# jenkinsm13/julia-spira

Hardware: AMD Instinct MI355X
Metric: Msamples/sec at 1920x1080 spp=64 depth=8; fraction of HBM roofline (higher is better)
Workload: dtype f64

## Files before the change

### julia-spira_amd/csrc/spira_device.h

```cpp
#pragma once
#include <hip/hip_runtime.h>
#include <stdint.h>
#include <type_traits>
#include "spira_fastdiv.h"

namespace spira {

__device__ __forceinline__ float sqrt_rn(float x) { return __builtin_sqrtf(x); }
__device__ __forceinline__ double sqrt_rn(double x) { return __builtin_sqrt(x); }

constexpr int kBlock = 256;
#ifndef SPIRA_WAVES_F32
#define SPIRA_WAVES_F32 5
#endif
#ifndef SPIRA_WAVES_F64
#define SPIRA_WAVES_F64 4
#endif
#define SPIRA_WAVES_PER_SIMD(T) (sizeof(T) == 8 ? SPIRA_WAVES_F64 : SPIRA_WAVES_F32)
constexpr uint32_t kMaxTries = 64;

template <class T> struct Vec { T x, y, z; };

template <class T> __device__ __forceinline__ Vec<T> mk(T x, T y, T z) { Vec<T> r; r.x = x; r.y = y; r.z = z; return r; }
template <class T> __device__ __forceinline__ Vec<T> operator+(Vec<T> a, Vec<T> b) { return mk<T>(a.x + b.x, a.y + b.y, a.z + b.z); }
// ... 870 lines not shown
template <class T>
__device__ __forceinline__ void dielectric_resolve(Pending<T> &pend, const Vec<T> d, const RngKey &key) {
    const Vec<T> n = pend.v;
    const T ior = pend.rough;
    const T cosd = dot(d, n);
    const bool entering = cosd < (T)0.0;
    const Vec<T> nn = entering ? n : mk<T>(-n.x, -n.y, -n.z);
    const T eta = entering ? (T)1.0 / ior : ior;
    const T ci = entering ? -cosd : cosd;
    const T s2 = (eta * eta) * ((T)1.0 - ci * ci);
    T r0 = ((T)1.0 - ior) / ((T)1.0 + ior); r0 = r0 * r0;
    const T x = (T)1.0 - ci, x2 = x * x;
    const T refl = r0 + ((T)1.0 - r0) * ((x2 * x2) * x);
    T u, u1, u2;
    rng3<T>(key, 1, u, u1, u2);
    if (s2 > (T)1.0 || u < refl) pend.v = d - nn * ((T)2 * dot(d, nn));
    else pend.v = d * eta + nn * (eta * ci - sqrt_rn((T)1.0 - s2));
    pend.kind = kMirror;
}

template <class T, bool BVH, bool EXT = false>
__device__ __forceinline__ SegInfo segment_front(const SceneLds<T> &sc, Vec<T> &o, const Vec<T> d, Vec<T> &beta, bool scatter,
                                                 Vec<T> &contrib, T &t_out, Pending<T> &pend, const ExtState<T> *ext = nullptr) {
    SegInfo info;
    T t;
    uint32_t slot;
    int prim = closest_hit<T, BVH>(sc, o, d, (T)0.001, t, slot);
    info.prim = prim;
    t_out = prim >= 0 ? t : (T)0;
    if (prim < 0) {
        pend.kind = kDead; pend.rough = 0; pend.v = mk<T>(0, 0, 0);
        contrib = sky_term_x<T, EXT>(d, beta, ext);
        info.alive = false; info.has_contrib = true;
        return info;
    }
    const Vec<T> pos = o + d * t;
    info.has_contrib = shade_hit<T, BVH, EXT>(sc, pos, d, prim, slot, beta, scatter, contrib, pend, ext);
    info.alive = scatter;
    if (scatter) o = pos;
    return info;
}

template <class T, class P>
__device__ __forceinline__ Vec<T> segment_back(const Vec<T> pos, const Pending<T> &pend, const Vec<T> rnd, P &pol) {
    if (pend.kind == kDiffuse) return normalize((pend.v + rnd) - pos, pol);
    Vec<T> reflected = pend.v;
    if (pend.kind == kSpecRough) reflected = reflected + rnd * pend.rough;
    return normalize(reflected, pol);
}
template <class T>
__device__ __forceinline__ Vec<T> segment_back(const Vec<T> pos, const Pending<T> &pend, const Vec<T> rnd) {
    ExactDiv exact;
    return segment_back<T>(pos, pend, rnd, exact);
}

template <class T, bool BVH, bool EXT = false>
__device__ __forceinline__ SegInfo trace_segment(const SceneLds<T> &sc, const RenderConst<T> &rc, Vec<T> &o, Vec<T> &d,
                                                 Vec<T> &beta, uint32_t pixel, uint32_t sample, uint32_t bounce,
                                                 bool scatter, Vec<T> &contrib, T &t_out, const ExtState<T> *ext = nullptr) {
    Pending<T> pend;
    const Vec<T> d_in = d;
    SegInfo info = segment_front<T, BVH, EXT>(sc, o, d, beta, scatter, contrib, t_out, pend, ext);
    if (info.alive) {
        Vec<T> rnd = mk<T>(0, 0, 0);
        if (EXT && pend.kind == kDielectric) dielectric_resolve<T>(pend, d_in, rng_key(rc.sA, rc.sB, pixel, sample, bounce));
        if (pend.kind == kDiffuse || pend.kind == kSpecRough)
            rnd = random_in_unit_sphere<T>(rng_key(rc.sA, rc.sB, pixel, sample, bounce));
        d = segment_back<T>(o, pend, rnd);
    }
    return info;
}

template <class T, class P>
__device__ __forceinline__ void camera_ray(const RenderConst<T> &rc, uint32_t i, uint32_t j, uint32_t pixel, uint32_t sample,
                                           Vec<T> &o, Vec<T> &d, P &pol) {
    T xu, xv, unused;
    rng3<T>(rng_key(rc.sA, rc.sB, pixel, sample, 0), 0, xu, xv, unused);
    T u = ((T)(i - 1) + xu) / (T)(rc.width - 1);
    T v = ((T)(j - 1) + xv) / (T)(rc.height - 1);
    o = rc.cam_origin;
    d = normalize(((rc.cam_llc + rc.cam_hor * u) + rc.cam_ver * v) - o, pol);
}
template <class T>
__device__ __forceinline__ void camera_ray(const RenderConst<T> &rc, uint32_t i, uint32_t j, uint32_t pixel, uint32_t sample,
                                           Vec<T> &o, Vec<T> &d) {
    ExactDiv exact;
    camera_ray<T>(rc, i, j, pixel, sample, o, d, exact);
}
__device__ __forceinline__ float to_scalar(float x) { return __uint_as_float(__builtin_amdgcn_readfirstlane(__float_as_uint(x))); }
__device__ __forceinline__ double to_scalar(double x) {
    const uint32_t lo = __builtin_amdgcn_readfirstlane((uint32_t)__double2loint(x)), hi = __builtin_amdgcn_readfirstlane((uint32_t)__double2hiint(x));
    return __hiloint2double((int)hi, (int)lo);
}
template <class T> struct PixelDiv { Recip<T> w1, h1; };
template <class T> __device__ __forceinline__ PixelDiv<T> pixel_divisors(const RenderConst<T> &rc) {
    PixelDiv<T> p;
    p.w1 = recip_of((T)(rc.width - 1)); p.h1 = recip_of((T)(rc.height - 1));
    p.w1.d = to_scalar(p.w1.d); p.w1.r = to_scalar(p.w1.r); p.h1.d = to_scalar(p.h1.d); p.h1.r = to_scalar(p.h1.r);
    return p;
}
template <class T> __device__ __forceinline__ T pixel_quotient(T n, const Recip<T> &rc, ExactDiv &) { return n / rc.d; }
template <class T> __device__ __forceinline__ T pixel_quotient(T n, const Recip<T> &rc, SpecDiv &) { return quotient(n, rc); }
template <class T, class P>
__device__ __forceinline__ void camera_ray_lds(const RenderConst<T> &rc, const T *cam, const PixelDiv<T> &pd, uint32_t i, uint32_t j, uint32_t pixel, uint32_t sample,
                                               Vec<T> &o, Vec<T> &d, P &pol) {
    T xu, xv, unused;
    rng3<T>(rng_key(rc.sA, rc.sB, pixel, sample, 0), 0, xu, xv, unused);
    T u = pixel_quotient<T>((T)(i - 1) + xu, pd.w1, pol);
    T v = pixel_quotient<T>((T)(j - 1) + xv, pd.h1, pol);
    o = mk<T>(cam[0], cam[1], cam[2]);
    const Vec<T> llc = mk<T>(cam[3], cam[4], cam[5]), hor = mk<T>(cam[6], cam[7], cam[8]), ver = mk<T>(cam[9], cam[10], cam[11]);
    d = normalize(((llc + hor * u) + ver * v) - o, pol);
}

template <class T>
__device__ __forceinline__ void path_of(const RenderConst<T> &rc, uint32_t q, uint32_t pass, uint32_t &i, uint32_t &j,
                                        uint32_t &pixel, uint32_t &sample) {
    uint32_t slot = fastdiv(q, rc.fd_tile);
    uint32_t pl = q - slot * rc.tile_pixels;
    uint32_t lr = fastdiv(pl, rc.fd_width);
    uint32_t lx = pl - lr * rc.width;
    j = ref_row_j(rc, lr);
    i = lx + 1;
    pixel = (j - 1) * rc.width + lx;
    sample = rc.sample0 + pass * rc.slots + slot;
}

template <class T> struct RayQueue { Pack4<T> *A; Pack4<T> *B; Pack2<T> *C; };

struct Stats {
    unsigned long long segments, rays_enqueued, radiance_rmw, radiance_store, redone_waves, rays_parked;
    unsigned long long mesh_wave_trips, mesh_lane_trips;
};

template <class T> struct BounceArgs {
    SceneGlobal<T> scene;
    RenderConst<T> rc;
    RayQueue<T> qin, qout;
    Pack3<T> *L;
    const uint32_t *cnt_in;
    uint32_t *cnt_out;
    uint32_t *blk_stats;
    uint32_t cap;
    Stats *stats;
    uint32_t bounce;
    uint32_t pass;
    uint32_t n_first;
};

__device__ __forceinline__ void wave_lds_sync() {
    __builtin_amdgcn_fence(__ATOMIC_RELEASE, "wavefront");
    __builtin_amdgcn_wave_barrier();
    __builtin_amdgcn_fence(__ATOMIC_ACQUIRE, "wavefront");
}

template <class T, bool FIRST, int R, bool BVH>
__global__ __launch_bounds__(kBlock, SPIRA_WAVES_PER_SIMD(T)) void k_bounce(const BounceArgs<T> a) {
    extern __shared__ __attribute__((aligned(32))) unsigned char lds_raw[];
    constexpr uint32_t WPB = kBlock / 64, SUB = 64 * R;
    const uint32_t lane = threadIdx.x & 63, wave = threadIdx.x >> 6;
    const uint32_t NW = gridDim.x * WPB, wid = blockIdx.x * WPB + wave;
    const RenderConst<T> &rc = a.rc;
    const bool scatter = (a.bounce + 1 < rc.max_depth);
    uint32_t n_mine = 0;
    if (!FIRST) {
        uint32_t n_blk = 0;
#pragma unroll
        for (uint32_t w = 0; w < WPB; ++w) n_blk += a.cnt_in[blockIdx.x * WPB + w];
        n_mine = a.cnt_in[wid];
        if (n_blk == 0) {
            if (lane == 0) { if (scatter) a.cnt_out[wid] = 0; a.blk_stats[4 * wid] = 0; a.blk_stats[4 * wid + 1] = 0; a.blk_stats[4 * wid + 2] = 0; a.blk_stats[4 * wid + 3] = 0; }
            return;
        }
    }
    const SceneLds<T> sc = stage_scene<T>(a.scene, lds_raw);
    Pack4<T> *s_rnd = reinterpret_cast<Pack4<T> *>(lds_raw + scene_lds_bytes<T>(a.scene.n_spheres, a.scene.n_materials, a.scene.n_triangles)) + wave * SUB;
    const uint32_t region = wid * a.cap;
    const unsigned long long lt_mask = (1ull << lane) - 1ull;
    uint32_t n_rmw = 0, n_store = 0, n_seg = 0, fill = 0;

    const uint32_t limit = FIRST ? a.n_first : n_mine;
    const uint32_t n_sub = (limit + SUB - 1) / SUB;
    for (uint32_t sub = FIRST ? wid : 0u; sub < n_sub; sub += FIRST ? NW : 1u) {
        Vec<T> o[R], beta[R];
        Pending<T> pend[R];
        uint32_t q[R], ent[R];
        uint32_t n_list = 0;
#pragma unroll
        for (int r = 0; r < R; ++r) {
            const uint32_t idx = sub * SUB + r * 64 + lane;
            pend[r].kind = kDead;
            bool want = false;
            RngKey key;
            if (idx < limit) {
                uint32_t pixel, sample, pi, pj;
                Vec<T> d;
                if (FIRST) {
                    q[r] = idx;
                    path_of<T>(rc, idx, a.pass, pi, pj, pixel, sample);
                    camera_ray<T>(rc, pi, pj, pixel, sample, o[r], d);
                    beta[r] = mk<T>(1, 1, 1);
                } else {
                    const Pack4<T> A = a.qin.A[region + idx], B = a.qin.B[region + idx];
                    const Pack2<T> C = a.qin.C[region + idx];
                    o[r] = mk<T>(A.x, A.y, A.z);
                    d = mk<T>(A.w, B.x, B.y);
                    beta[r] = mk<T>(B.z, B.w, C.x);
                    q[r] = Bits<T>::to_u32(C.y);
                }
                Vec<T> contrib; T t_hit;
                SegInfo si = segment_front<T, BVH>(sc, o[r], d, beta[r], scatter, contrib, t_hit, pend[r]);
                ++n_seg;
                const uint32_t qi = q[r] & 0x7FFFFFFFu;
                const bool has_l = (q[r] >> 31) != 0;
                if (si.has_contrib) {
                    Pack3<T> l; l.x = contrib.x; l.y = contrib.y; l.z = contrib.z;
                    if (has_l) { const Pack3<T> l0 = a.L[qi]; l.x = l0.x + contrib.x; l.y = l0.y + contrib.y; l.z = l0.z + contrib.z; ++n_rmw; }
                    else ++n_store;
                    a.L[qi] = l;
                    q[r] |= 0x80000000u;
                } else if (!si.alive && !has_l) {
                    Pack3<T> l; l.x = 0; l.y = 0; l.z = 0;
                    a.L[qi] = l;
                    ++n_store;
                }
                want = (pend[r].kind == kDiffuse || pend[r].kind == kSpecRough);
                if (want) {
                    if (!FIRST) path_of<T>(rc, qi, a.pass, pi, pj, pixel, sample);
                    key = rng_key(rc.sA, rc.sB, pixel, sample, a.bounce);
                }
            }
            if (scatter) {
                const unsigned long long m = __ballot(want);
                if (want) {
                    ent[r] = n_list + __popcll(m & lt_mask);
                    uint32_t *kw = reinterpret_cast<uint32_t *>(&s_rnd[ent[r]]);
                    kw[0] = key.hA; kw[1] = key.hB;
                }
                n_list += (uint32_t)__popcll(m);
            }
        }
        if (!scatter) continue;
        wave_lds_sync();
        {
            uint32_t e = lane, t = 1, next = 64;
            bool have = e < n_list;
            RngKey k; k.hA = 0; k.hB = 0; k.hBr = 0;
            if (have) {
                const uint32_t *kw = reinterpret_cast<const uint32_t *>(&s_rnd[e]);
                k.hA = kw[0]; k.hB = kw[1]; k.hBr = (k.hB << 16) | (k.hB >> 16);
            }
            while (__any(have)) {
                bool done = false;
                if (have) {
                    T u0, u1, u2;
                    rng3<T>(k, t, u0, u1, u2, (T)(1.0 / 1048576.0));
                    Vec<T> c = mk<T>(u0, u1, u2) - mk<T>(1, 1, 1);
                    done = dot(c, c) < (T)1.0;
                    if (!done && t == kMaxTries) { c = mk<T>(0, 0, 0); done = true; }
                    if (done) { Pack4<T> w; w.x = c.x; w.y = c.y; w.z = c.z; w.w = 0; s_rnd[e] = w; }
                    ++t;
                }
                const unsigned long long m = __ballot(done);
                if (done) {
                    e = next + __popcll(m & lt_mask); t = 1;
                    have = e < n_list;
                    if (have) {
                        const uint32_t *kw = reinterpret_cast<const uint32_t *>(&s_rnd[e]);
                        k.hA = kw[0]; k.hB = kw[1]; k.hBr = (k.hB << 16) | (k.hB >> 16);
                    }
                }
                next += (uint32_t)__popcll(m);
            }
        }
        wave_lds_sync();
#pragma unroll
        for (int r = 0; r < R; ++r) {
            const bool alive = pend[r].kind != kDead;
            const unsigned long long m = __ballot(alive);
            if (alive) {
                Vec<T> rnd = mk<T>(0, 0, 0);
                if (pend[r].kind != kMirror) { const Pack4<T> w = s_rnd[ent[r]]; rnd = mk<T>(w.x, w.y, w.z); }
                const Vec<T> nd = segment_back<T>(o[r], pend[r], rnd);
                const uint32_t dst = region + fill + __popcll(m & lt_mask);
                Pack4<T> A, B; Pack2<T> C;
                A.x = o[r].x; A.y = o[r].y; A.z = o[r].z; A.w = nd.x;
                B.x = nd.y; B.y = nd.z; B.z = beta[r].x; B.w = beta[r].y;
                C.x = beta[r].z; C.y = Bits<T>::from_u32(q[r]);
                a.qout.A[dst] = A; a.qout.B[dst] = B; a.qout.C[dst] = C;
            }
            fill += (uint32_t)__popcll(m);
        }
        wave_lds_sync();
    }
    for (int sft = 32; sft > 0; sft >>= 1) { n_rmw += __shfl_down(n_rmw, sft); n_seg += __shfl_down(n_seg, sft); n_store += __shfl_down(n_store, sft); }
    if (lane == 0) {
        if (scatter) a.cnt_out[wid] = fill;
        a.blk_stats[4 * wid] = n_seg;
        a.blk_stats[4 * wid + 1] = n_rmw;
        a.blk_stats[4 * wid + 2] = n_store;
        a.blk_stats[4 * wid + 3] = FIRST ? 0u : n_seg;
    }
}

template <class T> struct PathArgs {
    SceneGlobal<T> scene;
    RenderConst<T> rc;
    RayQueue<T> q[2];
    uint32_t *qref[2];
    uint2 *qkey[2];
    uint32_t cam_consts;
    Pack3<T> *L;
    uint32_t *blk_stats;
    uint32_t cap;
    uint32_t pass;
    uint32_t n_first;
    uint32_t dense_pct;
    Pack4<T> *mesh_list;
    uint32_t mesh_min_batch;
    uint32_t refill_free;
    uint32_t mesh_mode;
    uint32_t *mesh_count;
    uint32_t resume_k, resume_nw;
    uint32_t *redo;
    uint32_t redo_only;
    Stats *stats;
    Pack4<T> *accum;
    FastDiv fd_keff;
    uint32_t k_eff;
    uint32_t accum_first;
    uint32_t l_private;
};

#ifndef SPIRA_RESOLVE_RUN
#define SPIRA_RESOLVE_RUN 4
#endif
__device__ __forceinline__ uint32_t owned_pixel(uint32_t w, uint32_t nw, uint32_t l) {
    constexpr uint32_t kRun = SPIRA_RESOLVE_RUN;
    static_assert(64 % kRun == 0, "a run length divides the wave");
    return ((l / kRun) * nw + w) * kRun + l % kRun;
}

template <class T>
__device__ __forceinline__ void resolve_pixel(Pack4<T> *accum, const Pack3<T> *L, uint32_t tile_pixels, uint32_t k_eff, bool first_pass, uint32_t p) {
    Pack4<T> acc;
    if (first_pass) { acc.x = 0; acc.y = 0; acc.z = 0; acc.w = 0; } else acc = accum[p];
    uint32_t s = 0;
    for (; s + 8 <= k_eff; s += 8) {
        Pack3<T> l[8];
#pragma unroll
        for (int k = 0; k < 8; ++k) l[k] = L[(size_t)(s + k) * tile_pixels + p];
#pragma unroll
        for (int k = 0; k < 8; ++k) { acc.x = acc.x + l[k].x; acc.y = acc.y + l[k].y; acc.z = acc.z + l[k].z; }
    }
    for (; s < k_eff; ++s) {
        const Pack3<T> l = L[(size_t)s * tile_pixels + p];
        acc.x = acc.x + l.x; acc.y = acc.y + l.y; acc.z = acc.z + l.z;
    }
    accum[p] = acc;
}
template <class T>
__device__ __forceinline__ void resolve_pixel_run(Pack4<T> *accum, const Pack3<T> *Lp, uint32_t k_eff, bool first_pass, uint32_t p) {
    constexpr uint32_t kRun = SPIRA_RESOLVE_RUN;
    Pack4<T> acc;
    if (first_pass) { acc.x = 0; acc.y = 0; acc.z = 0; acc.w = 0; } else acc = accum[p];
    uint32_t s = 0;
    for (; s + 8 <= k_eff; s += 8) {
        Pack3<T> l[8];
#pragma unroll
        for (int k = 0; k < 8; ++k) l[k] = Lp[(s + k) * kRun];
#pragma unroll
        for (int k = 0; k < 8; ++k) { acc.x = acc.x + l[k].x; acc.y = acc.y + l[k].y; acc.z = acc.z + l[k].z; }
    }
    for (; s < k_eff; ++s) {
        const Pack3<T> l = Lp[s * kRun];
        acc.x = acc.x + l.x; acc.y = acc.y + l.y; acc.z = acc.z + l.z;
    }
    accum[p] = acc;
}

__device__ __forceinline__ float pack_qref(uint32_t q, uint32_t, float) { return __uint_as_float(q); }
__device__ __forceinline__ double pack_qref(uint32_t q, uint32_t ref, double) { return __longlong_as_double((long long)((unsigned long long)q | ((unsigned long long)ref << 32))); }
__device__ __forceinline__ uint32_t unpack_q(float w) { return __float_as_uint(w); }
__device__ __forceinline__ uint32_t unpack_q(double w) { return (uint32_t)(unsigned long long)__double_as_longlong(w); }
__device__ __forceinline__ uint32_t unpack_ref(double w) { return (uint32_t)((unsigned long long)__double_as_longlong(w) >> 32); }

#ifdef SPIRA_MESH_STATS
__device__ unsigned long long g_mesh_dbg[32];
#define MESH_STAT(...) __VA_ARGS__
#else
#define MESH_STAT(...)
#endif

#ifndef SPIRA_CARRY_KEY
#define SPIRA_CARRY_KEY 1
#endif
#ifndef SPIRA_WAVES_B_F32
#define SPIRA_WAVES_B_F32 4
#endif
#ifndef SPIRA_WAVES_B_F64
#define SPIRA_WAVES_B_F64 SPIRA_WAVES_F64
#endif
#ifndef SPIRA_WAVES_PATH_F32
#define SPIRA_WAVES_PATH_F32 6
#endif
template <class T, int R, bool BVH, bool EXT, bool SPEC, int MODE = 0, bool TRI = true>
__global__ __launch_bounds__(kBlock, MODE == 2 ? (sizeof(T) == 8 ? SPIRA_WAVES_B_F64 : SPIRA_WAVES_B_F32) : (sizeof(T) == 4 ? SPIRA_WAVES_PATH_F32 : SPIRA_WAVES_F64)) void k_path(const PathArgs<T> a) {
    extern __shared__ __attribute__((aligned(32))) unsigned char lds_raw[];
    constexpr uint32_t WPB = kBlock / 64, SUB = 64 * R;
    constexpr bool kRefArray = sizeof(T) == 4;
    constexpr bool kCarry = SPIRA_CARRY_KEY && !BVH && !EXT;
    constexpr uint32_t kStageShift = 25, kRefMask = (1u << kStageShift) - 1u;
    const uint32_t lane = threadIdx.x & 63, wave = threadIdx.x >> 6;
    const uint32_t NW = gridDim.x * WPB, wid = blockIdx.x * WPB + wave;
    const RenderConst<T> &rc = a.rc;
    using Pol = typename std::conditional<SPEC, SpecDiv, ExactDiv>::type;
    Pol pol;
    if (!SPEC && a.redo_only) {
        uint32_t any = 0;
        for (uint32_t w = 0; w < WPB; ++w) any |= a.redo[blockIdx.x * WPB + w];
        if (!any) return;
    }
    T *cam_lds = reinterpret_cast<T *>(lds_raw + scene_lds_bytes<T>(a.scene.n_spheres, a.scene.n_materials, a.scene.n_triangles) + WPB * SUB * sizeof(Pack4<T>));
    if (threadIdx.x < 12) {
        const Vec<T> *cv = threadIdx.x < 3 ? &rc.cam_origin : (threadIdx.x < 6 ? &rc.cam_llc : (threadIdx.x < 9 ? &rc.cam_hor : &rc.cam_ver));
        const uint32_t cc = threadIdx.x % 3;
        cam_lds[threadIdx.x] = cc == 0 ? cv->x : (cc == 1 ? cv->y : cv->z);
    }
    Pack4<T> *cam_sph = reinterpret_cast<Pack4<T> *>(reinterpret_cast<unsigned char *>(cam_lds) + 128);
    constexpr bool kCam = !EXT;
    if (kCam && MODE != 2 && a.cam_consts)
        for (uint32_t i = threadIdx.x; i < a.scene.n_spheres; i += blockDim.x) {
            const T *sp = a.scene.spheres5 + 5 * (size_t)i;
            const Vec<T> oc = rc.cam_origin - mk<T>(sp[0], sp[1], sp[2]);
            Pack4<T> k; k.x = oc.x; k.y = oc.y; k.z = oc.z; k.w = dot(oc, oc) - sp[3] * sp[3];
// ... 37 lines not shown
    uint32_t pfx[kMaxSeg + 1];
    bool segmented = false;
    {
        uint32_t cnt = 0;
        if (mesh_mode == 2u && lane < kseg && wid * kseg + lane < a.resume_nw) cnt = a.mesh_count[wid * kseg + lane];
        pfx[0] = 0;
#pragma unroll
        for (int j = 0; j < kMaxSeg; ++j) pfx[j + 1] = pfx[j] + (uint32_t)__builtin_amdgcn_readlane((int)cnt, j);
        if (mesh_mode == 2u) { mfill = pfx[kMaxSeg]; segmented = true; }
    }
    const uint32_t first_sub = own ? 0u : (mesh_mode == 1u ? (wid % a.resume_k) * (NW / a.resume_k) + wid / a.resume_k : wid);
    const uint32_t sub_step = own ? 1u : NW;
    MESH_STAT(unsigned long long dbg_t0 = __builtin_readcyclecounter(); unsigned long long dbg_sess = 0, dbg_walk = 0; uint32_t dbg_ns = 0, dbg_ws = 0, dbg_ls = 0, dbg_rf = 0, dbg_rays = 0, dbg_rounds = 0, dbg_ws1 = 0, dbg_ls1 = 0, dbg_h[4] = {0, 0, 0, 0};)
    for (uint32_t round = 0; ; ++round) {
        MESH_STAT(++dbg_rounds;)
        const bool first = mesh_mode != 2u && round == 0;
        const RayQueue<T> qin = a.q[(round + 1) & 1], qout = a.q[round & 1];
        const uint32_t *rin = a.qref[(round + 1) & 1];
        uint32_t *rout = a.qref[round & 1];
        const uint2 *kin = a.qkey[(round + 1) & 1];
        uint2 *kout = a.qkey[round & 1];
        const uint32_t limit = first ? (own ? n_own : a.n_first) : n_in;
        const uint32_t n_sub = first ? n_sub_first : (n_in + SUB - 1) / SUB;
        uint32_t fill = 0;
        for (uint32_t sub = first ? first_sub : 0u; sub < n_sub; sub += first ? sub_step : 1u) {
            Vec<T> o[R], beta[R];
            Pending<T> pend[R];
            ExtState<T> ex[R];
            uint32_t q[R], ent[R], stg[R], ref[R];
            uint32_t ka[R], kb[R];
            bool valid[R];
#pragma unroll
            for (int r = 0; r < R; ++r) {
                const uint32_t idx = sub * SUB + r * 64 + lane;
                valid[r] = false; stg[r] = round; ref[r] = 0; q[r] = 0; ka[r] = 0; kb[r] = 0;
                pend[r].kind = kDead; pend[r].rough = 0; pend[r].v = mk<T>(0, 0, 0);
                o[r] = mk<T>(0, 0, 0); beta[r] = mk<T>(1, 1, 1);
                bool parked = false; T park_t = 0; int park_prim = -1;
                uint32_t qf = idx;
                bool in = idx < limit;
                if (own && first) {
                    const uint32_t t = idx / SPIRA_RESOLVE_RUN, run = fastdiv(t, a.fd_keff);
                    const uint32_t px = owned_pixel(wid, NW, run * SPIRA_RESOLVE_RUN + idx % SPIRA_RESOLVE_RUN);
                    qf = (t - run * a.k_eff) * rc.tile_pixels + px;
                    in = in && px < rc.tile_pixels;
                }
                const uint32_t ql = priv ? l_base + idx : qf;
                if (in) {
                    if (first) {
                        uint32_t pixel, sample, pi, pj;
                        Vec<T> d;
                        q[r] = ql;
                        path_of<T>(rc, qf, a.pass, pi, pj, pixel, sample);
                        if (kCarry) { ka[r] = mix32(rc.sA + pixel) ^ (sample << 8); kb[r] = mix32(rc.sB ^ pixel) + (sample << 8); }
                        camera_ray_lds<T>(rc, cam_lds, pix_div, pi, pj, pixel, sample, o[r], d, pol);
                        if (EXT) { ex[r].flags = rc.flags; if (rc.flags & kExtSpectral) beta[r] = ext_wavelength<T>(sc, rc.sA, rc.sB, pixel, sample, ex[r]); }
                        T t; uint32_t slot = 0;
                        int prim;
                        if (defer) {
                            if (kCam && a.cam_consts) closest_hit_local<T, Pol, TRI, true>(sc, o[r], d, (T)0.001, t, prim, pol, cam_sph);
                            else closest_hit_local<T, Pol, TRI>(sc, o[r], d, (T)0.001, t, prim, pol);
                            parked = mesh_box_hit<T>(sc, o[r], d, t);
                        } else if (kCam && !BVH && a.cam_consts) { closest_hit_local<T, Pol, TRI, true>(sc, o[r], d, (T)0.001, t, prim, pol, cam_sph); }
                        else prim = closest_hit<T, BVH, Pol, TRI>(sc, o[r], d, (T)0.001, t, slot, pol);
                        ++n_seg;
                        if (parked) { park_t = t; park_prim = prim; pend[r].v = d; }
                        else if (prim < 0) {
                            const Vec<T> c = sky_term_x<T, EXT>(d, beta[r], &ex[r]);
                            Pack3<T> l; l.x = c.x; l.y = c.y; l.z = c.z;
                            a.L[ql] = l;
                            ++n_store;
                        } else {
                            valid[r] = true;
                            o[r] = o[r] + d * t;
                            ref[r] = (BVH && prim >= (int)ref_base) ? ref_base + slot : (uint32_t)prim;
                            pend[r].v = d;
                        }
                    } else {
                        const Pack4<T> A = qin.A[region + idx], B = qin.B[region + idx];
                        const Pack2<T> C = qin.C[region + idx];
                        o[r] = mk<T>(A.x, A.y, A.z);
                        pend[r].v = mk<T>(A.w, B.x, B.y);
                        beta[r] = mk<T>(B.z, B.w, C.x);
                        q[r] = unpack_q(C.y);
                        uint32_t w;
                        if constexpr (kRefArray) w = rin[region + idx]; else w = unpack_ref(C.y);
                        if (mixed) { stg[r] = w >> kStageShift; ref[r] = w & kRefMask; } else ref[r] = w;
                        if (kCarry) { const uint2 k = kin[region + idx]; ka[r] = k.x; kb[r] = k.y; }
                        valid[r] = true;
                    }
                }
                if (defer && first) {
                    const unsigned long long mp = __ballot(parked);
                    if (parked) park(mfill + __popcll(mp & lt_mask), o[r], pend[r].v, beta[r], park_t, q[r], park_prim, 0u);
                    mfill += (uint32_t)__popcll(mp); n_park += (uint32_t)__popcll(mp);
                }
            }
            while (true) {
                uint32_t n_list = 0, n_valid = 0;
#pragma unroll
                for (int r = 0; r < R; ++r) {
                    bool want = false;
                    RngKey key;
                    const Vec<T> d = pend[r].v;
                    pend[r].kind = kDead;
                    if (valid[r]) {
                        uint32_t pixel = 0, sample = 0, pi, pj;
                        const bool scatter = stg[r] + 1 < rc.max_depth;
                        int prim = (int)ref[r]; uint32_t slot = 0;
                        if (BVH && ref[r] >= ref_base) { prim = (int)ref_base; slot = ref[r] - ref_base; }
                        const uint32_t qi = q[r] & 0x7FFFFFFFu;
                        const bool has_l = (q[r] >> 31) != 0;
                        if (EXT) {
                            path_of<T>(rc, qi, a.pass, pi, pj, pixel, sample);
                            ex[r].flags = rc.flags;
                            if (rc.flags & kExtSpectral) (void)ext_wavelength<T>(sc, rc.sA, rc.sB, pixel, sample, ex[r]);
                        }
                        Vec<T> contrib;
                        const bool has_contrib = shade_hit<T, BVH, EXT, Pol, TRI>(sc, o[r], d, prim, slot, beta[r], scatter, contrib, pend[r], &ex[r], pol);
                        if (has_contrib) {
                            Pack3<T> l; l.x = contrib.x; l.y = contrib.y; l.z = contrib.z;
                            if (has_l) { const Pack3<T> l0 = a.L[qi]; l.x = l0.x + contrib.x; l.y = l0.y + contrib.y; l.z = l0.z + contrib.z; ++n_rmw; }
                            else ++n_store;
                            a.L[qi] = l;
                            q[r] |= 0x80000000u;
                        } else if (!scatter && !has_l) {
                            Pack3<T> l; l.x = 0; l.y = 0; l.z = 0;
                            a.L[qi] = l;
                            ++n_store;
                        }
                        want = (pend[r].kind == kDiffuse || pend[r].kind == kSpecRough);
                        if (want || (EXT && pend[r].kind == kDielectric)) {
                            if (kCarry && mixed) {
                                key.hA = mix32(ka[r] ^ stg[r]); key.hB = mix32(kb[r] + stg[r]); key.hBr = (key.hB << 16) | (key.hB >> 16);
                            } else {
                                if (!EXT) path_of<T>(rc, qi, a.pass, pi, pj, pixel, sample);
                                key = rng_key(rc.sA, rc.sB, pixel, sample, stg[r]);
                            }
                            if (EXT && pend[r].kind == kDielectric) dielectric_resolve<T>(pend[r], d, key);
                        }
                    }
                    const unsigned long long mv = __ballot(pend[r].kind != kDead);
                    n_valid += (uint32_t)__popcll(mv);
                    const unsigned long long m = __ballot(want);
                    if (want) {
                        ent[r] = n_list + __popcll(m & lt_mask);
                        uint32_t *kw = reinterpret_cast<uint32_t *>(&s_rnd[ent[r]]);
                        kw[0] = key.hA; kw[1] = key.hB;
                    }
                    n_list += (uint32_t)__popcll(m);
                }
                if (n_valid == 0) break;
                wave_lds_sync();
                {
                    uint32_t e = lane, t = 1, next = 64;
                    bool have = e < n_list;
                    RngKey k; k.hA = 0; k.hB = 0; k.hBr = 0;
                    if (have) {
                        const uint32_t *kw = reinterpret_cast<const uint32_t *>(&s_rnd[e]);
                        k.hA = kw[0]; k.hB = kw[1]; k.hBr = (k.hB << 16) | (k.hB >> 16);
                    }
                    while (__any(have)) {
                        bool done = false;
                        if (have) {
                            T u0, u1, u2;
                            rng3<T>(k, t, u0, u1, u2, (T)(1.0 / 1048576.0));
                            Vec<T> c = mk<T>(u0, u1, u2) - mk<T>(1, 1, 1);
                            done = dot(c, c) < (T)1.0;
                            if (!done && t == kMaxTries) { c = mk<T>(0, 0, 0); done = true; }
                            if (done) { Pack4<T> w; w.x = c.x; w.y = c.y; w.z = c.z; w.w = 0; s_rnd[e] = w; }
                            ++t;
                        }
                        const unsigned long long m = __ballot(done);
                        if (done) {
                            e = next + __popcll(m & lt_mask); t = 1;
                            have = e < n_list;
                            if (have) {
                                const uint32_t *kw = reinterpret_cast<const uint32_t *>(&s_rnd[e]);
                                k.hA = kw[0]; k.hB = kw[1]; k.hBr = (k.hB << 16) | (k.hB >> 16);
                            }
                        }
                        next += (uint32_t)__popcll(m);
                    }
                }
                wave_lds_sync();
                uint32_t n_hit = 0;
#pragma unroll
                for (int r = 0; r < R; ++r) {
                    bool hit = false, parked3 = false;
                    T park_t3 = 0; int park_prim3 = -1;
                    if (pend[r].kind != kDead) {
                        Vec<T> rnd = mk<T>(0, 0, 0);
                        if (pend[r].kind != kMirror) { const Pack4<T> w = s_rnd[ent[r]]; rnd = mk<T>(w.x, w.y, w.z); }
                        const Vec<T> nd = segment_back<T>(o[r], pend[r], rnd, pol);
                        T t; uint32_t slot = 0;
                        int prim;
                        if (defer) {
                            closest_hit_local<T, Pol, TRI>(sc, o[r], nd, (T)0.001, t, prim, pol);
                            parked3 = mesh_box_hit<T>(sc, o[r], nd, t);
                        } else prim = closest_hit<T, BVH, Pol, TRI>(sc, o[r], nd, (T)0.001, t, slot, pol);
                        ++n_seg;
                        if (parked3) { park_t3 = t; park_prim3 = prim; pend[r].v = nd; }
                        else if (prim < 0) {
                            const Vec<T> c = sky_term_x<T, EXT>(nd, beta[r], &ex[r]);
                            const uint32_t qi = q[r] & 0x7FFFFFFFu;
                            Pack3<T> l; l.x = c.x; l.y = c.y; l.z = c.z;
                            if (q[r] >> 31) { const Pack3<T> l0 = a.L[qi]; l.x = l0.x + c.x; l.y = l0.y + c.y; l.z = l0.z + c.z; ++n_rmw; }
                            else ++n_store;
                            a.L[qi] = l;
                        } else {
                            hit = true;
                            o[r] = o[r] + nd * t;
                            ref[r] = (BVH && prim >= (int)ref_base) ? ref_base + slot : (uint32_t)prim;
                            pend[r].v = nd;
                            ++stg[r];
                        }
                    }
                    if (defer) {
                        const unsigned long long mp = __ballot(parked3);
                        if (parked3) park(mfill + __popcll(mp & lt_mask), o[r], pend[r].v, beta[r], park_t3, q[r], park_prim3, stg[r] + 1u);
                        mfill += (uint32_t)__popcll(mp); n_park += (uint32_t)__popcll(mp);
                    }
                    valid[r] = hit;
                    n_hit += (uint32_t)__popcll(__ballot(hit));
                }
                wave_lds_sync();
                if (n_hit == 0) break;
                if (dense_pct && n_hit * 100u >= n_valid * dense_pct) continue;
#pragma unroll
                for (int r = 0; r < R; ++r) {
                    const unsigned long long m = __ballot(valid[r]);
                    if (valid[r]) {
                        const uint32_t dst = region + fill + __popcll(m & lt_mask);
                        const Vec<T> nd = pend[r].v;
                        const uint32_t w = mixed ? (ref[r] | (stg[r] << kStageShift)) : ref[r];
                        Pack4<T> A, B; Pack2<T> C;
                        A.x = o[r].x; A.y = o[r].y; A.z = o[r].z; A.w = nd.x;
                        B.x = nd.y; B.y = nd.z; B.z = beta[r].x; B.w = beta[r].y;
                        C.x = beta[r].z; C.y = pack_qref(q[r], w, (T)0);
                        qout.A[dst] = A; qout.B[dst] = B; qout.C[dst] = C;
                        if constexpr (kRefArray) rout[dst] = w;
                        if constexpr (kCarry) kout[dst] = make_uint2(ka[r], kb[r]);
                    }
                    fill += (uint32_t)__popcll(m);
                }
                break;
            }
        }
        if (defer && mesh_mode != 1u && mfill && (mfill >= a.mesh_min_batch || fill == 0)) {
            constexpr int kLdsStack = (int)(SUB * sizeof(Pack4<T>) / (64 * sizeof(uint32_t)));
            __builtin_amdgcn_fence(__ATOMIC_RELEASE, "workgroup");
            __builtin_amdgcn_fence(__ATOMIC_ACQUIRE, "workgroup");
            uint32_t *lstack = reinterpret_cast<uint32_t *>(s_rnd);
            uint32_t stack[kBvhStackD - kLdsStack];
            uint32_t next = 0;
            MESH_STAT(const unsigned long long dbg_s0 = __builtin_readcyclecounter(); ++dbg_ns; dbg_rays += mfill;)
#ifdef SPIRA_BVH_SCREEN
            constexpr bool kScreened = sizeof(T) == 8;
#else
            constexpr bool kScreened = false;
#endif
            if constexpr (kScreened) {
            bool walking = false, finished = false, full = false;
            uint32_t ent_i = 0;
            float dxf = 0, dyf = 0, dzf = 1;
            Bvh8Ray ry; ry.ox = ry.oy = ry.oz = 0; ry.ix = ry.iy = ry.iz = 1; ry.oct = 0; ry.best = 0; ry.tmin = 0; ry.amin = 0;
            Bvh8Walk<T> wk; wk.G = 0; wk.tw = 0; wk.rank = 0; wk.sp = 0; wk.t0 = 0; wk.c0 = wk.c1 = wk.c2 = wk.c3 = 0; wk.nc = 0;
            auto decode = [&](const Pack4<T> A, const Pack4<T> B, const Pack4<T> C, Vec<T> &o_, Vec<T> &d_, Vec<T> &beta_, T &closest, uint32_t &q_, int &prim, uint32_t &slot, uint32_t &stage_hit) {
                o_ = mk<T>(A.x, A.y, A.z); d_ = mk<T>(A.w, B.x, B.y); beta_ = mk<T>(B.z, B.w, C.x);
                closest = C.y;
                q_ = Bits<T>::to_u32(C.z);
                const uint32_t pw = Bits<T>::to_u32(C.w);
                prim = (int)(pw & kRefMask) - 1;
                stage_hit = pw >> kStageShift;
                slot = 0;
                if (prim >= (int)ref_base) { slot = (uint32_t)prim - ref_base; prim = (int)ref_base; }
            };
            while (true) {
                if (__any(full)) {
                    if (full) {
                        Pack4<T> *ent = a.mesh_list + 3 * (size_t)ent_i;
                        const Pack4<T> A = ent[0], B = ent[1];
                        Pack4<T> C = ent[2];
                        Vec<T> o_, d_, beta_; T closest; uint32_t q_, slot, stage_hit; int prim;
                        decode(A, B, C, o_, d_, beta_, closest, q_, prim, slot, stage_hit);
                        while (wk.nc) bvh8_resolve_one<T>(sc, wk, ry, o_, d_, (T)0.001, (int)ref_base, closest, prim, slot);
                        C.y = closest;
                        C.w = Bits<T>::from_u32((uint32_t)((prim >= (int)ref_base ? (int)(ref_base + slot) : prim) + 1) | (stage_hit << kStageShift));
                        ent[2] = C;
                        full = false;
                    }
                    __builtin_amdgcn_fence(__ATOMIC_RELEASE, "workgroup");
                    __builtin_amdgcn_fence(__ATOMIC_ACQUIRE, "workgroup");
                }
                {
                    Vec<T> o_ = mk<T>(0, 0, 0), d_ = mk<T>(0, 0, 1), beta_ = mk<T>(0, 0, 0);
                    T closest = 0; uint32_t q_ = 0, stage_hit = 0, slot = 0; int prim = -1;
                    if (finished) {
                        const Pack4<T> *ent = a.mesh_list + 3 * (size_t)ent_i;
                        const bool has = wk.nc != 0;
                        const uint32_t ti = has ? wk.c0 : 0u;
                        const Pack4<T> *rec = sc.bvh_tris + 3 * (size_t)ti;
                        const Pack4<T> A = ent[0], B = ent[1], C = ent[2];
                        const Pack4<T> v0 = rec[0], e1 = rec[1], e2 = rec[2];
                        decode(A, B, C, o_, d_, beta_, closest, q_, prim, slot, stage_hit);
                        if (has) {
                            wk.c0 = wk.c1; wk.c1 = wk.c2; wk.c2 = wk.c3; --wk.nc;
                            T t;
                            if (triangle_test<T>(v0, e1, e2, o_, d_, (T)0.001, closest, t)) {
                                const int p = (int)ref_base + (int)Bits<T>::to_u32(v0.w);
                                if (t < closest || p > prim) { closest = t; prim = p; slot = ti; }
                            }
                        }
                    }
                    while (__any(finished && wk.nc != 0)) {
                        if (finished && wk.nc != 0) bvh8_resolve_one<T>(sc, wk, ry, o_, d_, (T)0.001, (int)ref_base, closest, prim, slot);
                    }
                    const unsigned long long mh = __ballot(finished && prim >= 0);
                    if (finished) {
                        if (prim < 0) {
                            const uint32_t qi = q_ & 0x7FFFFFFFu;
                            ExtState<T> ex1; ex1.flags = rc.flags; ex1.bR = 0; ex1.bG = 0; ex1.bB = 0;
                            if (EXT && (rc.flags & kExtSpectral)) {
                                uint32_t pi, pj, pixel, sample;
                                path_of<T>(rc, qi, a.pass, pi, pj, pixel, sample);
                                (void)ext_wavelength<T>(sc, rc.sA, rc.sB, pixel, sample, ex1);
                            }
                            const Vec<T> c = sky_term_x<T, EXT>(d_, beta_, &ex1);
                            Pack3<T> l; l.x = c.x; l.y = c.y; l.z = c.z;
                            if (q_ >> 31) { const Pack3<T> l0 = a.L[qi]; l.x = l0.x + c.x; l.y = l0.y + c.y; l.z = l0.z + c.z; ++n_rmw; }
                            else ++n_store;
                            a.L[qi] = l;
                        } else {
                            const Vec<T> hp = o_ + d_ * closest;
                            const uint32_t w_ = ((prim >= (int)ref_base) ? ref_base + slot : (uint32_t)prim) | (stage_hit << kStageShift);
                            const uint32_t dst = region + fill + __popcll(mh & lt_mask);
                            Pack4<T> A, B; Pack2<T> C;
                            A.x = hp.x; A.y = hp.y; A.z = hp.z; A.w = d_.x;
                            B.x = d_.y; B.y = d_.z; B.z = beta_.x; B.w = beta_.y;
                            C.x = beta_.z; C.y = pack_qref(q_, w_, (T)0);
                            qout.A[dst] = A; qout.B[dst] = B; qout.C[dst] = C;
                            if constexpr (kRefArray) rout[dst] = w_;
                        }
                    }
                    fill += (uint32_t)__popcll(mh);
                    finished = false;
// ... 975 lines not shown
```

Measured before the change: 27570.

## Drain unit-sphere rejection tail with lane groups and integer acceptance test

Moves the per-wave rejection-sampling drain into a shared helper. Once the list nears empty, the helper spreads the remaining entries' successive tries across groups of lanes, so the tail takes fewer wave iterations. For f64, the acceptance test runs in 64-bit integer arithmetic on the raw hash words, and only the two words are stored in LDS, to be converted to doubles when read. The tail adds LDS table writes, extra syncs and ballot bit work. Python emulators are included to check the results match the serial version exactly.

```diff
diff --git a/julia-spira_amd/csrc/spira_device.h b/julia-spira_amd/csrc/spira_device.h
--- a/julia-spira_amd/csrc/spira_device.h
+++ b/julia-spira_amd/csrc/spira_device.h
@@ -1046,6 +1046,123 @@
     __builtin_amdgcn_fence(__ATOMIC_RELEASE, "wavefront");
     __builtin_amdgcn_wave_barrier();
     __builtin_amdgcn_fence(__ATOMIC_ACQUIRE, "wavefront");
+}
+
+#ifndef SPIRA_RND_TAIL
+#define SPIRA_RND_TAIL 1
+#endif
+#ifndef SPIRA_RND_INT
+#define SPIRA_RND_INT 1
+#endif
+template <class T> constexpr bool kRndPacked = SPIRA_RND_INT && sizeof(T) == 8;
+
+template <class T, bool PACKED = kRndPacked<T>> struct RndTry {
+    Vec<T> c;
+    __device__ __forceinline__ bool draw(const RngKey &k, uint32_t t) {
+        T u0, u1, u2;
+        rng3<T>(k, t, u0, u1, u2, (T)(1.0 / 1048576.0));
+        c = mk<T>(u0, u1, u2) - mk<T>(1, 1, 1);
+        return dot(c, c) < (T)1.0;
+    }
+    __device__ __forceinline__ void zero() { c = mk<T>(0, 0, 0); }
+    __device__ __forceinline__ void store(Pack4<T> *slot) const { Pack4<T> w; w.x = c.x; w.y = c.y; w.z = c.z; w.w = 0; *slot = w; }
+    static __device__ __forceinline__ Vec<T> load(const Pack4<T> *slot) { const Pack4<T> w = *slot; return mk<T>(w.x, w.y, w.z); }
+};
+template <class T> struct RndTry<T, true> {
+    uint32_t a, b;
+    __device__ __forceinline__ bool draw(const RngKey &k, uint32_t t) {
+        a = mix32((k.hA + t * 0x9E3779B9u) ^ k.hBr);
+        b = mix32(a + k.hB);
+        const int32_t k0 = (int32_t)(a >> 11) - (1 << 20), k1 = (int32_t)(b >> 11) - (1 << 20);
+        const int32_t k2 = (int32_t)(((a & 0x7FFu) << 10) | (b & 0x3FFu)) - (1 << 20);
+        const uint64_t s = (uint64_t)((int64_t)k0 * k0) + (uint64_t)((int64_t)k1 * k1) + (uint64_t)((int64_t)k2 * k2);
+        return s < (1ull << 40);
+    }
+    __device__ __forceinline__ void zero() { a = 0x80000400u; b = 0x80000000u; }
+    __device__ __forceinline__ void store(Pack4<T> *slot) const { *reinterpret_cast<uint2 *>(slot) = make_uint2(a, b); }
+    static __device__ __forceinline__ Vec<T> load(const Pack4<T> *slot) {
+        const uint2 w = *reinterpret_cast<const uint2 *>(slot);
+        const T s = (T)(1.0 / 1048576.0);
+        const T u0 = (T)(w.x >> 11) * s, u1 = (T)(w.y >> 11) * s, u2 = (T)(((w.x & 0x7FFu) << 10) | (w.y & 0x3FFu)) * s;
+        return mk<T>(u0, u1, u2) - mk<T>(1, 1, 1);
+    }
+};
+
+template <class T, uint32_t MAXT = kMaxTries>
+__device__ __forceinline__ void drain_unit_sphere_list(Pack4<T> *s_rnd, uint32_t n_list, uint32_t lane) {
+    const unsigned long long lt_mask = (1ull << lane) - 1ull;
+    uint32_t e = lane, t = 1, next = 64;
+    bool have = e < n_list;
+    RngKey k; k.hA = 0; k.hB = 0; k.hBr = 0;
+    if (have) {
+        const uint32_t *kw = reinterpret_cast<const uint32_t *>(&s_rnd[e]);
+        k.hA = kw[0]; k.hB = kw[1]; k.hBr = (k.hB << 16) | (k.hB >> 16);
+    }
+#if SPIRA_RND_TAIL
+    unsigned long long pm = __ballot(have);
+    while (pm != 0 && (next < n_list || __popcll(pm) > 32)) {
+#else
+    while (__any(have)) {
+#endif
+        bool done = false;
+        if (have) {
+            RndTry<T> r;
+            done = r.draw(k, t);
+            if (!done && t == MAXT) { r.zero(); done = true; }
+            if (done) r.store(&s_rnd[e]);
+            ++t;
+        }
+        const unsigned long long m = __ballot(done);
+        if (done) {
+            e = next + __popcll(m & lt_mask); t = 1;
+            have = e < n_list;
+            if (have) {
+                const uint32_t *kw = reinterpret_cast<const uint32_t *>(&s_rnd[e]);
+                k.hA = kw[0]; k.hB = kw[1]; k.hBr = (k.hB << 16) | (k.hB >> 16);
+            }
+        }
+        next += (uint32_t)__popcll(m);
+#if SPIRA_RND_TAIL
+        pm = __ballot(have);
+#endif
+    }
+#if SPIRA_RND_TAIL
+    constexpr uint32_t kSlotWords = sizeof(Pack4<T>) / 4;
+    uint32_t *tab = reinterpret_cast<uint32_t *>(s_rnd) + (kSlotWords - 1);
+    uint32_t p = (uint32_t)__popcll(pm), lg = ~0u;
+    bool lead = have;
+    while (p != 0) {
+        const uint32_t lg_new = min(5u, 6u - (32u - (uint32_t)__clz((int)(p - 1))));
+        if (lg_new != lg) {
+            lg = lg_new;
+            if (lead) tab[kSlotWords * (uint32_t)__popcll(pm & lt_mask)] = e | (t << 16);
+            wave_lds_sync();
+            const uint32_t grp = lane >> lg;
+            have = grp < p;
+            if (have) {
+                const uint32_t w = tab[kSlotWords * grp];
+                e = w & 0xFFFFu; t = w >> 16;
+                const uint32_t *kw = reinterpret_cast<const uint32_t *>(&s_rnd[e]);
+                k.hA = kw[0]; k.hB = kw[1]; k.hBr = (k.hB << 16) | (k.hB >> 16);
+            }
+        }
+        const uint32_t g = 1u << lg, j = lane & (g - 1u);
+        RndTry<T> r;
+        bool acc = false;
+        if (have && t + j <= MAXT) acc = r.draw(k, t + j);
+        const unsigned long long m = __ballot(acc);
+        const uint32_t half = lane < 32u ? (uint32_t)m : (uint32_t)(m >> 32);
+        const uint32_t field = (half >> ((lane & 31u) - j)) & (0xFFFFFFFFu >> (32u - g));
+        if (acc && (field & ((1u << j) - 1u)) == 0u) r.store(&s_rnd[e]);
+        const bool over = field == 0u && t + g > MAXT;
+        if (have && over && j == 0u) { r.zero(); r.store(&s_rnd[e]); }
+        have = have && field == 0u && !over;
+        t += g;
+        lead = have && j == 0u;
+        pm = __ballot(lead);
+        p = (uint32_t)__popcll(pm);
+    }
+#endif
 }
 
 template <class T, bool FIRST, int R, bool BVH>
@@ -1136,37 +1253,7 @@
         }
         if (!scatter) continue;
         wave_lds_sync();
-        {
-            uint32_t e = lane, t = 1, next = 64;
-            bool have = e < n_list;
-            RngKey k; k.hA = 0; k.hB = 0; k.hBr = 0;
-            if (have) {
-                const uint32_t *kw = reinterpret_cast<const uint32_t *>(&s_rnd[e]);
-                k.hA = kw[0]; k.hB = kw[1]; k.hBr = (k.hB << 16) | (k.hB >> 16);
-            }
-            while (__any(have)) {
-                bool done = false;
-                if (have) {
-                    T u0, u1, u2;
-                    rng3<T>(k, t, u0, u1, u2, (T)(1.0 / 1048576.0));
-                    Vec<T> c = mk<T>(u0, u1, u2) - mk<T>(1, 1, 1);
-                    done = dot(c, c) < (T)1.0;
-                    if (!done && t == kMaxTries) { c = mk<T>(0, 0, 0); done = true; }
-                    if (done) { Pack4<T> w; w.x = c.x; w.y = c.y; w.z = c.z; w.w = 0; s_rnd[e] = w; }
-                    ++t;
-                }
-                const unsigned long long m = __ballot(done);
-                if (done) {
-                    e = next + __popcll(m & lt_mask); t = 1;
-                    have = e < n_list;
-                    if (have) {
-                        const uint32_t *kw = reinterpret_cast<const uint32_t *>(&s_rnd[e]);
-                        k.hA = kw[0]; k.hB = kw[1]; k.hBr = (k.hB << 16) | (k.hB >> 16);
-                    }
-                }
-                next += (uint32_t)__popcll(m);
-            }
-        }
+        drain_unit_sphere_list<T>(s_rnd, n_list, lane);
         wave_lds_sync();
 #pragma unroll
         for (int r = 0; r < R; ++r) {
@@ -1174,7 +1261,7 @@
             const unsigned long long m = __ballot(alive);
             if (alive) {
                 Vec<T> rnd = mk<T>(0, 0, 0);
-                if (pend[r].kind != kMirror) { const Pack4<T> w = s_rnd[ent[r]]; rnd = mk<T>(w.x, w.y, w.z); }
+                if (pend[r].kind != kMirror) rnd = RndTry<T>::load(&s_rnd[ent[r]]);
                 const Vec<T> nd = segment_back<T>(o[r], pend[r], rnd);
                 const uint32_t dst = region + fill + __popcll(m & lt_mask);
                 Pack4<T> A, B; Pack2<T> C;
@@ -1518,37 +1605,7 @@
                 }
                 if (n_valid == 0) break;
                 wave_lds_sync();
-                {
-                    uint32_t e = lane, t = 1, next = 64;
-                    bool have = e < n_list;
-                    RngKey k; k.hA = 0; k.hB = 0; k.hBr = 0;
-                    if (have) {
-                        const uint32_t *kw = reinterpret_cast<const uint32_t *>(&s_rnd[e]);
-                        k.hA = kw[0]; k.hB = kw[1]; k.hBr = (k.hB << 16) | (k.hB >> 16);
-                    }
-                    while (__any(have)) {
-                        bool done = false;
-                        if (have) {
-                            T u0, u1, u2;
-                            rng3<T>(k, t, u0, u1, u2, (T)(1.0 / 1048576.0));
-                            Vec<T> c = mk<T>(u0, u1, u2) - mk<T>(1, 1, 1);
-                            done = dot(c, c) < (T)1.0;
-                            if (!done && t == kMaxTries) { c = mk<T>(0, 0, 0); done = true; }
-                            if (done) { Pack4<T> w; w.x = c.x; w.y = c.y; w.z = c.z; w.w = 0; s_rnd[e] = w; }
-                            ++t;
-                        }
-                        const unsigned long long m = __ballot(done);
-                        if (done) {
-                            e = next + __popcll(m & lt_mask); t = 1;
-                            have = e < n_list;
-                            if (have) {
-                                const uint32_t *kw = reinterpret_cast<const uint32_t *>(&s_rnd[e]);
-                                k.hA = kw[0]; k.hB = kw[1]; k.hBr = (k.hB << 16) | (k.hB >> 16);
-                            }
-                        }
-                        next += (uint32_t)__popcll(m);
-                    }
-                }
+                drain_unit_sphere_list<T>(s_rnd, n_list, lane);
                 wave_lds_sync();
                 uint32_t n_hit = 0;
 #pragma unroll
@@ -1557,7 +1614,7 @@
                     T park_t3 = 0; int park_prim3 = -1;
                     if (pend[r].kind != kDead) {
                         Vec<T> rnd = mk<T>(0, 0, 0);
-                        if (pend[r].kind != kMirror) { const Pack4<T> w = s_rnd[ent[r]]; rnd = mk<T>(w.x, w.y, w.z); }
+                        if (pend[r].kind != kMirror) rnd = RndTry<T>::load(&s_rnd[ent[r]]);
                         const Vec<T> nd = segment_back<T>(o[r], pend[r], rnd, pol);
                         T t; uint32_t slot = 0;
                         int prim;
diff --git a/profiles/experiments/rnd_list_drain_emul.py b/profiles/experiments/rnd_list_drain_emul.py
--- /dev/null
+++ b/profiles/experiments/rnd_list_drain_emul.py
@@ -0,0 +1,115 @@
+import numpy as np, sys
+M32 = 0xFFFFFFFF
+def mix32(x):
+    x = np.asarray(x, dtype=np.uint64) & M32
+    x ^= x >> 16; x = (x * 0x7feb352d) & M32
+    x ^= x >> 15; x = (x * 0x846ca68b) & M32
+    x ^= x >> 16
+    return x
+def words(hA, hB, t):
+    hBr = ((hB << 16) | (hB >> 16)) & M32
+    a = mix32(((hA + t * 0x9E3779B9) & M32) ^ hBr)
+    b = mix32((a + hB) & M32)
+    return a, b
+def ms(a, b):
+    return (a >> 11).astype(np.int64), (b >> 11).astype(np.int64), (((a & 0x7FF) << 10) | (b & 0x3FF)).astype(np.int64)
+def acc_int(a, b):
+    m0, m1, m2 = ms(a, b)
+    k0, k1, k2 = m0 - (1 << 20), m1 - (1 << 20), m2 - (1 << 20)
+    return (k0 * k0 + k1 * k1 + k2 * k2) < (1 << 40)
+def acc_f64(a, b):
+    m0, m1, m2 = ms(a, b)
+    s = 1.0 / 1048576.0
+    c0, c1, c2 = m0 * s - 1.0, m1 * s - 1.0, m2 * s - 1.0
+    return (c0 * c0 + c1 * c1 + c2 * c2) < 1.0
+def serial(hA, hB, maxt):
+    for t in range(1, maxt + 1):
+        a, b = words(np.uint64(hA), np.uint64(hB), t)
+        if acc_int(a, b): return (int(a), int(b))
+    return (0x80000400, 0x80000000)
+def popc(x): return bin(x).count("1")
+def drain(keys, maxt):
+    n = len(keys)
+    slot = [dict(k=keys[i] if i < n else None, res=None, tab=None) for i in range(128)]
+    lane = list(range(64))
+    e = list(range(64)); t = [1] * 64; nxt = 64
+    have = [x < n for x in e]
+    k = [slot[x]["k"] if have[i] else (0, 0) for i, x in enumerate(e)]
+    def draw(i, tt):
+        a, b = words(np.uint64(k[i][0]), np.uint64(k[i][1]), tt)
+        return bool(acc_int(a, b)), (int(a), int(b))
+    iters = 0
+    pm = [i for i in lane if have[i]]
+    while pm and (nxt < n or len(pm) > 32):
+        iters += 1
+        done = [False] * 64
+        for i in lane:
+            if have[i]:
+                d, r = draw(i, t[i])
+                if not d and t[i] == maxt: r = (0x80000400, 0x80000000); d = True
+                if d:
+                    assert slot[e[i]]["res"] is None; slot[e[i]]["res"] = r
+                t[i] += 1
+                done[i] = d
+        m = [i for i in lane if done[i]]
+        for i in m:
+            e[i] = nxt + sum(1 for x in m if x < i); t[i] = 1
+            have[i] = e[i] < n
+            if have[i]: k[i] = slot[e[i]]["k"]
+        nxt += len(m)
+        pm = [i for i in lane if have[i]]
+    p = len(pm); lg = None
+    lead = list(have)
+    while p:
+        iters += 1
+        cl = 32 - (32 - (p - 1).bit_length()) if p > 1 else 0
+        lg_new = min(5, 6 - cl)
+        if lg_new != lg:
+            lg = lg_new
+            for i in lane:
+                if lead[i]: slot[sum(1 for x in pm if x < i)]["tab"] = e[i] | (t[i] << 16)
+            for i in lane:
+                grp = i >> lg
+                have[i] = grp < p
+                if have[i]:
+                    w = slot[grp]["tab"]; e[i] = w & 0xFFFF; t[i] = w >> 16; k[i] = slot[e[i]]["k"]
+        g = 1 << lg
+        assert g * p <= 64
+        acc = [False] * 64; r = [None] * 64
+        for i in lane:
+            j = i & (g - 1)
+            if have[i] and t[i] + j <= maxt: acc[i], r[i] = draw(i, t[i] + j)
+        mbits = sum(1 << i for i in lane if acc[i])
+        newhave = list(have)
+        for i in lane:
+            j = i & (g - 1)
+            half = (mbits & M32) if i < 32 else (mbits >> 32)
+            field = (half >> ((i & 31) - j)) & (M32 >> (32 - g))
+            if acc[i] and (field & ((1 << j) - 1)) == 0:
+                assert slot[e[i]]["res"] is None; slot[e[i]]["res"] = r[i]
+            over = field == 0 and t[i] + g > maxt
+            if have[i] and over and j == 0:
+                assert slot[e[i]]["res"] is None; slot[e[i]]["res"] = (0x80000400, 0x80000000)
+            newhave[i] = have[i] and field == 0 and not over
+            t[i] += g
+            lead[i] = newhave[i] and j == 0
+        have = newhave
+        pm = [i for i in lane if lead[i]]
+        p = len(pm)
+    return [s["res"] for s in slot[:n]], iters
+rng = np.random.default_rng(1)
+a = rng.integers(0, 1 << 32, 2_000_000, dtype=np.uint64); b = rng.integers(0, 1 << 32, 2_000_000, dtype=np.uint64)
+assert np.array_equal(acc_int(a, b), acc_f64(a, b)); print("int == f64 accept on 2e6 draws, accept rate %.4f" % acc_int(a, b).mean())
+m0, m1, m2 = ms(np.uint64(0x80000400), np.uint64(0x80000000)); assert m0 == m1 == m2 == 1 << 20
+bad = 0
+for maxt in (64, 1, 2, 3, 5, 7):
+    ex = ok = 0
+    for n in (0, 1, 2, 3, 31, 32, 33, 63, 64, 65, 127, 128):
+        for rep in range(6):
+            keys = [(int(x), int(y)) for x, y in rng.integers(0, 1 << 32, (n, 2), dtype=np.uint64)]
+            got, it = drain(keys, maxt)
+            want = [serial(x, y, maxt) for x, y in keys]
+            if got != want: bad += 1; print("MISMATCH", maxt, n)
+            ex += sum(1 for w in want if w == (0x80000400, 0x80000000)); ok += sum(1 for w in want if w != (0x80000400, 0x80000000))
+    print("MAXT", maxt, "exhausted", ex, "accepted", ok)
+print("bad", bad)
diff --git a/profiles/experiments/rnd_list_drain_sim.py b/profiles/experiments/rnd_list_drain_sim.py
--- /dev/null
+++ b/profiles/experiments/rnd_list_drain_sim.py
@@ -0,0 +1,92 @@
+#!/usr/bin/env python3
+import math
+import random
+import sys
+
+P = math.pi / 6
+LENGTHS = (128, 100, 64, 32, 16, 8, 4, 1)
+
+
+def serial(acc, maxt):
+    return [next((t for t in range(1, maxt + 1) if a[t]), 0) for a in acc]
+
+
+def drain(acc, maxt, rule):
+    n = len(acc)
+    res = [None] * n
+    lanes = [(e, 1) for e in range(min(n, 64))]
+    nxt, iters, tries = 64, 0, 0
+    while lanes and (rule == "one" or nxt < n or len(lanes) > 32):
+        iters += 1
+        tries += len(lanes)
+        keep = []
+        for e, t in lanes:
+            if acc[e][t] or t == maxt:
+                res[e] = t if acc[e][t] else 0
+                if nxt < n:
+                    keep.append((nxt, 1))
+                    nxt += 1
+            else:
+                keep.append((e, t + 1))
+        lanes = keep
+    pend = lanes
+    g = 0
+    while pend:
+        p = len(pend)
+        g_new = 1 << int(math.log2(64 // p))
+        if rule == "built":
+            g_new = min(g_new, 32)
+            if g_new != g:
+                g, groups = g_new, list(pend)
+        else:
+            g, groups = g_new, list(pend)
+        iters += 1
+        out = []
+        for grp in groups:
+            if grp is None:
+                out.append(None)
+                continue
+            e, t0 = grp
+            span = [t for t in range(t0, t0 + g) if t <= maxt]
+            tries += len(span)
+            hit = next((t for t in span if acc[e][t]), 0)
+            if hit or t0 + g > maxt:
+                res[e] = hit
+                out.append(None)
+            else:
+                out.append((e, t0 + g))
+        groups = out
+        pend = [x for x in groups if x is not None]
+    return iters, tries, res
+
+
+def main():
+    lists = int(sys.argv[1]) if len(sys.argv) > 1 else 4000
+    maxt = int(sys.argv[2]) if len(sys.argv) > 2 else 64
+    rng = random.Random(20261017)
+    rows = {r: [] for r in ("one", "issue", "built")}
+    util = {r: [] for r in rows}
+    for n in LENGTHS:
+        tot = {r: [0, 0] for r in rows}
+        for _ in range(lists):
+            acc = [[False] + [rng.random() < P for _ in range(maxt + 32)] for _ in range(n)]
+            want = serial(acc, maxt)
+            for r in rows:
+                it, tr, res = drain(acc, maxt, r)
+                assert res == want, (r, n)
+                tot[r][0] += it
+                tot[r][1] += tr
+        for r in rows:
+            rows[r].append(tot[r][0] / lists)
+            util[r].append(tot[r][1] / (64.0 * tot[r][0]))
+    print("| entries on the list | " + " | ".join(str(n) for n in LENGTHS) + " |")
+    print("|---|" + "---:|" * len(LENGTHS))
+    for r, label in (("one", "iterations, one lane per entry"), ("issue", "iterations, group tries re-formed every iteration"), ("built", "iterations, as built")):
+        print("| %s | " % label + " | ".join("%.1f" % v for v in rows[r]) + " |")
+    print("| lanes evaluating a try, one lane per entry | " + " | ".join("%.2f" % v for v in util["one"]) + " |")
+    print("| lanes evaluating a try, as built | " + " | ".join("%.2f" % v for v in util["built"]) + " |")
+    print("| ideal (n / (pi/6) / 64) | " + " | ".join("%.2f" % (n / P / 64) for n in LENGTHS) + " |")
+
+
+if __name__ == "__main__":
+    main()
```

New measurement: 28390, median of 6. 1.03x the previous value.
